# treangenlab/Seqwin

Measured on AMD Instinct MI355X. Metric: Gbp/s minimizer-indexed, higher is better.
Workload: dtype u64

## Files before the change

### seqwin_amd/csrc/device.hpp

```cpp
#pragma once

#include <hip/hip_runtime.h>

#include <functional>
#include <memory>
#include <string>

#include "common.hpp"

namespace sw {

#define SW_HIP(expr)                                                                                   \
    do {                                                                                               \
        hipError_t _e = (expr);                                                                        \
        if (_e != hipSuccess)                                                                          \
            ::sw::raise(SW_ERR_DEVICE, "HIP error %d (%s) at %s:%d: %s", (int)_e, hipGetErrorString(_e), \
                        __FILE__, __LINE__, #expr);                                                    \
    } while (0)

__host__ __device__ inline uint64_t mix64(uint64_t x)
{
    x ^= x >> 30; x *= 0xbf58476d1ce4e5b9ULL;
    x ^= x >> 27; x *= 0x94d049bb133111ebULL;
    x ^= x >> 31;
// ... 181 lines not shown
};
std::vector<int> devices_from_env();
void build_multi_device(const char *const *paths, size_t n_paths, uint64_t k, uint64_t w, uint64_t n_cpu, std::vector<int> devs,
                        MultiGraph &out, uint64_t chunk_bp = 0);

Plan &get_plan(sw_batch &b, uint64_t k, uint64_t w, bool *cached = nullptr);

struct SketchOut {
    DevArray<uint64_t> stage_hash;
    DevArray<uint64_t> stage_kmer;
    DevArray<uint32_t> tile_count;
    DevArray<uint64_t> tile_offset;
    uint64_t n_occ = 0;
    uint64_t launches = 0;
    uint64_t n_ovf_tiles = 0;
};
void run_sketch(const sw_batch &b, const Plan &plan, hipStream_t stream, SketchOut &out, float *sketch_ms);

void radix_sort_keys64(uint64_t *&keys, uint64_t *&alt, uint64_t n, unsigned begin_bit, unsigned end_bit, hipStream_t stream,
                       uint32_t *d_fail, bool perm_hi32 = false, unsigned long long *d_hist_given = nullptr, unsigned layout_bits = 0);
void radix_layout(unsigned bits, unsigned *digit_bits, unsigned *n_passes);
bool radix_unsort_perm(uint64_t *&keys, uint64_t *&alt, uint64_t n, unsigned low_bits, unsigned nbit, hipStream_t stream, uint32_t *d_fail);
constexpr uint32_t UNSORT_CURSOR_STRIDE = 32;
struct UnsortPerm {
    DevArray<unsigned long long> cur_a, cur_b;
    DevArray<uint32_t> tickets;
    unsigned low_bits = 0, hi_bits = 0;
    uint32_t n_groups = 0, n_tiles = 0, grid = 0;
};
bool radix_unsort_perm_begin(UnsortPerm &u, uint64_t n, unsigned low_bits, unsigned nbit, hipStream_t stream);
void radix_unsort_perm_first(UnsortPerm &u, const uint64_t *keys, uint64_t *alt, uint64_t n, hipStream_t stream, uint32_t *d_fail);
void radix_unsort_perm_second(UnsortPerm &u, const uint64_t *keys, uint64_t *alt, uint64_t n, hipStream_t stream, uint32_t *d_fail);

int radix_edge_buckets(uint64_t *&keys, uint64_t *&alt, uint64_t m, unsigned key_bits, uint64_t sentinel,
                       const unsigned long long *d_hist_top, uint32_t cap, uint32_t slots, uint64_t *ukeys, uint32_t *ucnt,
                       uint32_t *n_runs, hipStream_t stream, uint32_t *d_fail, bool debug);

void sort_keys64(uint64_t *&keys, uint64_t *&keys_alt, size_t n, unsigned begin_bit, unsigned end_bit, hipStream_t stream,
                 uint32_t *d_fail, bool perm_hi32 = false, unsigned long long *d_hist_given = nullptr, unsigned layout_bits = 0);
bool sort_keys64_is_own(size_t n);
void check_sort_failed(uint32_t fail_word);

struct alignas(16) OccPay {
    uint32_t low, pos, rec, idx;
};
int radix_rank_mode();
bool radix_pairs_available();
uint64_t radix_trim_state();
void radix_demote_rank();
constexpr uint32_t STAGE_WIN = 32;
constexpr uint32_t STAGE_ROW = STAGE_WIN + 9;
constexpr uint32_t STAGE_PAD = 1;
struct StageSource {
    const uint64_t *stage_hash, *stage_kmer;
    const uint32_t *tile_count;
    const uint64_t *tile_offset;
    const uint64_t *dst_off;
    uint32_t n_tiles;
    uint64_t mult;
    uint32_t *rec_out;
    const unsigned long long *chunk_dir;
    const uint64_t *rows;
};
void radix_sort_pairs32(uint32_t *&keys, uint32_t *&keys_alt, OccPay *&vals, OccPay *&vals_alt, uint64_t n, unsigned end_bit,
                        hipStream_t stream, uint32_t *d_fail, const StageSource *src = nullptr,
                        const std::function<void()> &after_first = std::function<void()>(), uint32_t *low_out = nullptr);
bool sort_pairs32(uint32_t *&keys, uint32_t *&keys_alt, OccPay *&vals, OccPay *&vals_alt, uint64_t n, unsigned end_bit,
                  hipStream_t stream, uint32_t *d_fail, uint32_t *low_out = nullptr);
struct PartState;
// ... 80 lines not shown
```

### seqwin_amd/csrc/index.hip

```cpp
#include <cstdlib>
#include <cstring>
#include <map>
#include <memory>

#include <rocprim/rocprim.hpp>

#include "device.hpp"

namespace sw {

namespace {

constexpr int TPB = 256;
inline unsigned blocks_for(uint64_t n, int per = TPB) { return (unsigned)((n + per - 1) / per); }
inline bool ranks_by_table()
{
    const char *e = SW_TEST_GETENV("SEQWIN_AMD_RANKS");
    return e && !strcmp(e, "table");
}

template <class K, class V>
void sort_pairs(K *&keys, K *&keys_alt, V *&vals, V *&vals_alt, size_t n, unsigned begin_bit, unsigned end_bit,
                hipStream_t stream)
{
// ... 1160 lines not shown
                                  unsigned hi_bits, uint64_t lo_base, const RankHash H, sw_edge *__restrict__ edges)
{
    const uint64_t e = (uint64_t)blockIdx.x * blockDim.x + threadIdx.x;
    if (e >= n_edges) return;
    const uint64_t key = ukeys[e];
    const uint64_t u = (hi_bits >= 64 ? 0ull : (key >> hi_bits)) + lo_base;
    const uint64_t v = hi_bits >= 64 ? key : (key & ((1ull << hi_bits) - 1ull));
    edges[e].first = H(u);
    edges[e].second = H(v);
    edges[e].weight = RUNS ? usum[e + 1] - usum[e] : usum[e];
}

struct RepeatFlag {
    const uint64_t *keys;
    const uint32_t *vals;
    __host__ __device__ uint32_t operator()(uint64_t s) const
    {
        return (s && keys[s] == keys[s - 1] && vals[s] == vals[s - 1]) ? 1u : 0u;
    }
};

__global__ void k_subtract_repeats(const uint64_t *__restrict__ rkeys, const uint32_t *__restrict__ rdups, uint32_t n_runs,
                                   const uint64_t *__restrict__ ukeys, uint64_t n_edges, sw_edge *__restrict__ edges)
{
    const uint32_t i = blockIdx.x * blockDim.x + threadIdx.x;
    if (i >= n_runs || rdups[i] == 0) return;
    const uint64_t key = rkeys[i];
    uint64_t lo = 0, hi = n_edges;
    while (lo < hi) {
        const uint64_t mid = (lo + hi) >> 1;
        if (ukeys[mid] < key) lo = mid + 1; else hi = mid;
    }
    if (lo < n_edges && ukeys[lo] == key) edges[lo].weight -= rdups[i];
}

struct AsmChangeAny {
    const uint64_t *keys;
    const uint32_t *vals;
    __host__ __device__ uint32_t operator()(uint64_t s) const
    {
        return (s == 0 || keys[s] != keys[s - 1] || vals[s] != vals[s - 1]) ? 1u : 0u;
    }
};

__global__ void k_check_ascending(const uint64_t *__restrict__ keys, uint64_t m, uint32_t *__restrict__ order_bad)
{
    const uint64_t i = (uint64_t)blockIdx.x * blockDim.x + threadIdx.x;
    if (i && i < m && keys[i] < keys[i - 1]) atomicAdd(order_bad, 1u);
}

__global__ void k_drop_sentinel_run(const uint64_t *__restrict__ ukeys, uint64_t sentinel, uint32_t *__restrict__ count)
{
    const uint32_t n = *count;
    if (n && ukeys[n - 1] == sentinel) *count = n - 1;
}

constexpr int RLE_THREADS = 1024, RLE_ITEMS = 8;
constexpr uint32_t RLE_TILE = RLE_THREADS * RLE_ITEMS;
__global__ __launch_bounds__(RLE_THREADS) void k_rle_keys(const uint64_t *__restrict__ keys, uint64_t m, uint64_t *__restrict__ ukeys,
                                                           uint32_t *__restrict__ ustart, unsigned long long *__restrict__ tile_state,
                                                           uint32_t *__restrict__ ticket, uint32_t *__restrict__ n_runs_out,
                                                           uint32_t *__restrict__ order_bad)
{
    __shared__ uint32_t s_tile, s_excl, s_wave[RLE_THREADS / 64];
    __shared__ uint64_t s_last[RLE_THREADS / 64];
    const uint32_t lane = threadIdx.x & 63u, wave = threadIdx.x >> 6;
// ... 1705 lines not shown
    SW_HIP(hipGetLastError());
    SW_HIP(hipStreamSynchronize(stream));
}
}

namespace {
constexpr uint64_t EDGE_BUCKET_MIN_KEYS = 1ull << 26;
constexpr uint32_t EDGE_BUCKET_CAP = 1u << 20, EDGE_BUCKET_SLOTS = 4096;
struct WideKeys {
    unsigned lo_bits, hi_bits;
    uint64_t lo_base;
    RankHash hash;
};
void edges_from_pairs(uint64_t *keys, uint64_t *keys_alt, uint64_t m, uint64_t sentinel, unsigned nb, unsigned ab,
                      uint64_t *ck, uint32_t *ca, const unsigned long long *d_n_cand, uint64_t host_n_cand,
                      const uint64_t *rank_hash, hipStream_t stream, sw_index &ix, hipEvent_t rank_hash_ready = nullptr,
                      unsigned long long *d_hist = nullptr, const WideKeys *wide = nullptr)
{
    ix.n_edges = 0;
    if (m == 0) return;
    const unsigned key_bits = wide ? wide->lo_bits + wide->hi_bits : 2 * nb;
    DevArray<uint32_t> sort_fail(1);
    SW_HIP(hipMemsetAsync(sort_fail.p, 0, 4, stream));
    unsigned low_bits = 0, skip = 0, digit_bits = 0, n_passes = 0;
    if (sort_keys64_is_own(m)) {
        radix_layout(key_bits, &digit_bits, &n_passes);
        const unsigned hb = wide ? wide->hi_bits : nb;
        skip = hb >= digit_bits + 8 ? 1 : 0;
        if (skip && hb >= 2 * digit_bits + 8 && ix.n_nodes && m <= 4 * ix.n_nodes) skip = 2;
        if (const char *e = SW_TEST_GETENV("SEQWIN_AMD_EDGE_SKIP_PASSES")) skip = (unsigned)atoi(e);
        skip = std::min(skip, n_passes - 1);
        low_bits = skip * digit_bits;
    }
    DevArray<uint64_t> ukeys(m);
    DevArray<uint32_t> ucnt(m + 1), ucount(2);
    unsigned long long n_cand = host_n_cand;
    const char *rle_env = SW_AB_GETENV("SEQWIN_AMD_RLE");
    const bool own_rle = !(rle_env && !strcmp(rle_env, "rocprim"));
    bool by_buckets = !wide && nb < 32 && own_rle && sort_keys64_is_own(m) && m >= EDGE_BUCKET_MIN_KEYS && ix.n_nodes && m > 4 * ix.n_nodes;
    uint32_t bucket_cap = EDGE_BUCKET_CAP, bucket_slots = EDGE_BUCKET_SLOTS;
    if (const char *e = SW_TEST_GETENV("SEQWIN_AMD_EDGE_SORT")) by_buckets = !wide && nb < 32 && own_rle && !strcmp(e, "bucket");
    if (const char *e = SW_TEST_GETENV("SEQWIN_AMD_EDGE_BUCKET_CAP")) bucket_cap = (uint32_t)strtoul(e, nullptr, 10);
    if (const char *e = SW_TEST_GETENV("SEQWIN_AMD_EDGE_BUCKET_SLOTS")) bucket_slots = (uint32_t)strtoul(e, nullptr, 10);
    if (by_buckets) {
        unsigned db = 0, np = 0;
        radix_layout(key_bits, &db, &np);
        uint32_t n_runs = 0;
        by_buckets = radix_edge_buckets(keys, keys_alt, m, key_bits, sentinel, d_hist ? d_hist + ((size_t)(np - 1) << db) : nullptr, bucket_cap,
                                        bucket_slots, ukeys.p, ucnt.p, &n_runs, stream, sort_fail.p,
                                        getenv("SEQWIN_AMD_DEBUG_EDGE_REPAIR") != nullptr) == 0;
        if (by_buckets) {
            uint32_t failed = 0;
            SW_HIP(hipMemcpyAsync(&failed, sort_fail.p, 4, hipMemcpyDeviceToHost, stream));
            if (d_n_cand) SW_HIP(hipMemcpyAsync(&n_cand, d_n_cand, 8, hipMemcpyDeviceToHost, stream));
            SW_HIP(hipStreamSynchronize(stream));
            check_sort_failed(failed);
            ix.n_edges = n_runs;
        }
    }
    if (!by_buckets)
        sort_keys64(keys, keys_alt, m, low_bits, key_bits, stream, sort_fail.p, false,
                    d_hist ? d_hist + ((size_t)skip << digit_bits) : nullptr, key_bits);
    RepairState rep;
    if (low_bits && !by_buckets) enqueue_repair(EdgeKeyView{keys, low_bits}, EdgeKeyView{keys, low_bits}, ~0ull, m, nullptr, 0, rep, stream);
    bool demoted = false;
    for (int attempt = 0; !by_buckets; ++attempt) {
        SW_HIP(hipMemsetAsync(ucount.p + 1, 0, 4, stream));
        if (own_rle) {
            const unsigned blocks = (unsigned)((m + RLE_TILE - 1) / RLE_TILE);
            DevArray<unsigned long long> tile_state(blocks);
            DevArray<uint32_t> ticket(1);
            SW_HIP(hipMemsetAsync(tile_state.p, 0, (size_t)blocks * 8, stream));
            SW_HIP(hipMemsetAsync(ticket.p, 0, 4, stream));
            hipLaunchKernelGGL(k_rle_keys, dim3(blocks), dim3(RLE_THREADS), 0, stream, (const uint64_t *)keys, m, ukeys.p, ucnt.p, tile_state.p,
                               ticket.p, ucount.p, ucount.p + 1);
            SW_HIP(hipGetLastError());
        } else {
#ifdef SW_AB
            hipLaunchKernelGGL(k_check_ascending, dim3(blocks_for(m)), dim3(TPB), 0, stream, (const uint64_t *)keys, m, ucount.p + 1);
            size_t tmp_bytes = 0;
            SW_HIP(rocprim::run_length_encode(nullptr, tmp_bytes, keys, m, ukeys.p, ucnt.p, ucount.p, stream));
            DevArray<unsigned char> tmp(tmp_bytes);
            SW_HIP(rocprim::run_length_encode(tmp.p, tmp_bytes, keys, m, ukeys.p, ucnt.p, ucount.p, stream));
            SW_HIP(hipStreamSynchronize(stream));
#endif
        }
        hipLaunchKernelGGL(k_drop_sentinel_run, dim3(1), dim3(1), 0, stream, ukeys.p, sentinel, ucount.p);
        SW_HIP(hipGetLastError());
        uint32_t n_edges = 0, failed = 0, left = 0, descents = 0;
        SW_HIP(hipMemcpyAsync(&n_edges, ucount.p, 4, hipMemcpyDeviceToHost, stream));
        SW_HIP(hipMemcpyAsync(&descents, ucount.p + 1, 4, hipMemcpyDeviceToHost, stream));
        SW_HIP(hipMemcpyAsync(&failed, sort_fail.p, 4, hipMemcpyDeviceToHost, stream));
        if (low_bits && attempt == 0) SW_HIP(hipMemcpyAsync(&left, rep.status.p, 4, hipMemcpyDeviceToHost, stream));
        if (d_n_cand) SW_HIP(hipMemcpyAsync(&n_cand, d_n_cand, 8, hipMemcpyDeviceToHost, stream));
        SW_HIP(hipStreamSynchronize(stream));
        check_sort_failed(failed);
        if (low_bits && attempt == 0 && getenv("SEQWIN_AMD_DEBUG_EDGE_REPAIR")) {
            unsigned long long nd[2] = {0, 0};
            uint32_t st[2] = {0, 0};
            SW_HIP(hipMemcpy(nd, rep.n_desc.p, 16, hipMemcpyDeviceToHost));
            SW_HIP(hipMemcpy(st, rep.status.p, 8, hipMemcpyDeviceToHost));
            fprintf(stderr, "[edge repair] %llu keys, %u low bits: %llu descents, %u long runs, leftovers %u\n", (unsigned long long)m, low_bits,
                    nd[0], st[1], st[0]);
        }
        if (left) {
            sort_keys64(keys, keys_alt, m, 0, key_bits, stream, sort_fail.p);
            continue;
        }
        if (descents) {
            if (demoted)
                raise(SW_ERR_RUNTIME, "internal error: the edge keys are still out of order after the ballot-ranked re-sort (%u places)", descents);
            order_guard_tripped(1, descents);
            radix_demote_rank();
            demoted = true;
            sort_keys64(keys, keys_alt, m, 0, key_bits, stream, sort_fail.p);
            continue;
        }
        ix.n_edges = n_edges;
        break;
    }
    if (ix.n_edges == 0) return;
    ix.edges.alloc(ix.n_edges);
    if (rank_hash_ready) SW_HIP(hipStreamWaitEvent(stream, rank_hash_ready, 0));
    if (wide && own_rle)
        hipLaunchKernelGGL(k_edges_runs_wide<true>, dim3(blocks_for(ix.n_edges)), dim3(TPB), 0, stream, ukeys.p, ucnt.p, (uint64_t)ix.n_edges,
                           wide->hi_bits, wide->lo_base, wide->hash, ix.edges.p);
    else if (wide)
        hipLaunchKernelGGL(k_edges_runs_wide<false>, dim3(blocks_for(ix.n_edges)), dim3(TPB), 0, stream, ukeys.p, ucnt.p, (uint64_t)ix.n_edges,
                           wide->hi_bits, wide->lo_base, wide->hash, ix.edges.p);
    else if (own_rle)
        hipLaunchKernelGGL(k_edges_runs<true>, dim3(blocks_for(ix.n_edges)), dim3(TPB), 0, stream, ukeys.p, ucnt.p, 0u, ~0ull,
                           (uint64_t)ix.n_edges, nb, ix.nodes.p, rank_hash, ix.edges.p);
    else
        hipLaunchKernelGGL(k_edges_runs<false>, dim3(blocks_for(ix.n_edges)), dim3(TPB), 0, stream, ukeys.p, ucnt.p, 0u, ~0ull,
                           (uint64_t)ix.n_edges, nb, ix.nodes.p, rank_hash, ix.edges.p);
    SW_HIP(hipGetLastError());
    if (n_cand) {
        const uint64_t c = n_cand;
        DevArray<uint64_t> ck1(c);
        DevArray<uint32_t> ca1(c);
        uint32_t *a = ca, *a_alt = ca1.p;
        uint64_t *k = ck, *k_alt = ck1.p;
        sort_pairs(a, a_alt, k, k_alt, c, 0, ab, stream);
        sort_pairs(k, k_alt, a, a_alt, c, 0, key_bits, stream);
        DevArray<uint64_t> rkeys(c);
        DevArray<uint32_t> rdups(c), rcount(1);
        auto flags = rocprim::make_transform_iterator(rocprim::make_counting_iterator<uint64_t>(0), RepeatFlag{k, a});
        size_t tmp_bytes = 0;
        SW_HIP(rocprim::reduce_by_key(nullptr, tmp_bytes, k, flags, c, rkeys.p, rdups.p, rcount.p, rocprim::plus<uint32_t>(),
                                      rocprim::equal_to<uint64_t>(), stream));
        DevArray<unsigned char> tmp(tmp_bytes);
        SW_HIP(rocprim::reduce_by_key(tmp.p, tmp_bytes, k, flags, c, rkeys.p, rdups.p, rcount.p, rocprim::plus<uint32_t>(),
                                      rocprim::equal_to<uint64_t>(), stream));
        uint32_t n_runs = 0;
        SW_HIP(hipMemcpyAsync(&n_runs, rcount.p, 4, hipMemcpyDeviceToHost, stream));
        SW_HIP(hipStreamSynchronize(stream));
        if (n_runs) {
            hipLaunchKernelGGL(k_subtract_repeats, dim3(blocks_for(n_runs)), dim3(TPB), 0, stream, rkeys.p, rdups.p, n_runs, ukeys.p,
                               (uint64_t)ix.n_edges, ix.edges.p);
            SW_HIP(hipGetLastError());
        }
    }
    SW_HIP(hipStreamSynchronize(stream));
}

void edges_from_adjacency(uint64_t *keys, uint64_t *keys_alt, uint32_t *vals, uint32_t *vals_alt, uint64_t m,
                          uint64_t sentinel, unsigned nb, const uint64_t *rank_hash, hipStream_t stream, sw_index &ix)
{
    ix.n_edges = 0;
    if (m == 0) return;
    sort_pairs(keys, keys_alt, vals, vals_alt, m, 0, 2 * nb, stream);
    DevArray<uint64_t> ukeys(m);
    DevArray<uint32_t> usum(m);
    DevArray<uint32_t> ucount(1);
    {
        auto flags = rocprim::make_transform_iterator(rocprim::make_counting_iterator<uint64_t>(0), AsmChangeAny{keys, vals});
        size_t tmp_bytes = 0;
        SW_HIP(rocprim::reduce_by_key(nullptr, tmp_bytes, keys, flags, m, ukeys.p, usum.p, ucount.p, rocprim::plus<uint32_t>(),
                                      rocprim::equal_to<uint64_t>(), stream));
        DevArray<unsigned char> tmp(tmp_bytes);
        SW_HIP(rocprim::reduce_by_key(tmp.p, tmp_bytes, keys, flags, m, ukeys.p, usum.p, ucount.p, rocprim::plus<uint32_t>(),
                                      rocprim::equal_to<uint64_t>(), stream));
        hipLaunchKernelGGL(k_drop_sentinel_run, dim3(1), dim3(1), 0, stream, ukeys.p, sentinel, ucount.p);
        SW_HIP(hipGetLastError());
        uint32_t n_edges = 0;
        SW_HIP(hipMemcpyAsync(&n_edges, ucount.p, 4, hipMemcpyDeviceToHost, stream));
        SW_HIP(hipStreamSynchronize(stream));
        ix.n_edges = n_edges;
    }
    if (ix.n_edges == 0) return;
    ix.edges.alloc(ix.n_edges);
    hipLaunchKernelGGL(k_edges_runs<false>, dim3(blocks_for(ix.n_edges)), dim3(TPB), 0, stream, ukeys.p, usum.p, 0u, ~0ull,
                       (uint64_t)ix.n_edges, nb, ix.nodes.p, rank_hash, ix.edges.p);
    SW_HIP(hipGetLastError());
    SW_HIP(hipStreamSynchronize(stream));
}
// ... 1028 lines not shown
```

### seqwin_amd/csrc/radix.hip

```cpp
#include <algorithm>
#include <cstdlib>
#include <cstring>
#include <vector>
#include <map>
#include <mutex>

#include "device.hpp"

namespace sw {
namespace {

constexpr int RS_ITEMS = 16;
#ifdef SW_RS_STAMPS
__device__ unsigned long long *g_rs_stamps = nullptr;
#define RS_STAMP(i)                                                                                        \
    do {                                                                                                   \
        if (g_rs_stamps && (tile & 63u) == 0 && threadIdx.x == 0) g_rs_stamps[(size_t)(tile >> 6) * 16 + (i)] = clock64(); \
    } while (0)
#else
#define RS_STAMP(i) do { } while (0)
#endif
#ifndef RS_LOOK
#define RS_LOOK 4
#endif
// ... 1427 lines not shown
    }
}

#ifdef SW_RS_STAMPS
__device__ unsigned long long *g_eb_stamps = nullptr;
constexpr uint32_t EB_ST_EVERY = 16, EB_ST_WORDS = 16;
#define EB_STAMP(i) do { if (st) st[i] = clock64(); } while (0)
#define EB_STAMP_ADD(i, since) do { if (st) { const unsigned long long t_ = clock64(); st[i] += t_ - (since); (since) = t_; } } while (0)
#else
#define EB_STAMP(i) do { } while (0)
#define EB_STAMP_ADD(i, since) do { } while (0)
#endif

template <bool PACKED>
__global__ __launch_bounds__(EB_THREADS) void k_eb_finish(const uint64_t *__restrict__ in, const uint4 *__restrict__ live, uint32_t slots,
                                                          unsigned shift1, unsigned shift2, uint32_t mask2, unsigned bin_shift,
                                                          uint32_t bin_mask, unsigned cb, uint64_t sentinel,
                                                          uint64_t *__restrict__ tk, uint32_t *__restrict__ tc,
                                                          uint32_t *__restrict__ n_distinct, uint32_t *__restrict__ flags)
{
    extern __shared__ __align__(16) unsigned char eb_lds[];
    unsigned long long *hk = reinterpret_cast<unsigned long long *>(eb_lds);
    uint32_t *hc = reinterpret_cast<uint32_t *>(hk + slots);
    uint16_t *idx = PACKED ? reinterpret_cast<uint16_t *>(hk + slots) : reinterpret_cast<uint16_t *>(hc + slots);
    __shared__ uint32_t bd[EB_RADIX + 1], bk[EB_RADIX], bcur[EB_RADIX], wsd[EB_THREADS / 64], wsk[EB_THREADS / 64];
    __shared__ uint32_t s_over;
    const uint32_t tid = threadIdx.x, lane = tid & 63u, wave = tid >> 6;
#ifdef SW_RS_STAMPS
    unsigned long long *st = g_eb_stamps && tid == 0 && blockIdx.x % EB_ST_EVERY == 0 ? g_eb_stamps + (size_t)(blockIdx.x / EB_ST_EVERY) * EB_ST_WORDS : nullptr;
    unsigned long long st_t = 0;
#endif
    EB_STAMP(0);
    const uint4 me = live[blockIdx.x];
    const uint32_t mask = slots - 1u;
    for (uint32_t s = tid; s < slots; s += EB_THREADS) {
        hk[s] = EB_EMPTY;
        if (!PACKED) hc[s] = 0;
    }
    bd[tid] = 0;
    bk[tid] = 0;
    if (tid == 0) s_over = 0;
    const uint32_t b = me.x, first = me.y, cnt = me.z;
    const uint64_t low_mask = (1ull << shift2) - 1ull, count_mask = (1ull << cb) - 1ull;
    const uint64_t high = ((uint64_t)(b / EB_RADIX) << shift1) | ((uint64_t)(b % EB_RADIX) << shift2);
    uint64_t nxt[4];
#pragma unroll
    for (int i = 0; i < 4; ++i) {
        const uint32_t j = i * EB_THREADS + tid;
        nxt[i] = j < cnt ? in[(uint64_t)first + j] : sentinel;
    }
    EB_STAMP(1);
    __syncthreads();
    EB_STAMP(2);
#ifdef SW_RS_STAMPS
    if (st) st_t = clock64();
#endif
    uint32_t bad = 0;
    for (uint32_t j0 = 0; j0 < cnt; j0 += 4 * EB_THREADS) {
        if (*(volatile uint32_t *)&s_over) break;
        uint64_t key[4];
#pragma unroll
        for (int i = 0; i < 4; ++i) key[i] = nxt[i];
        if (j0 + 4 * EB_THREADS < cnt) {
#pragma unroll
            for (int i = 0; i < 4; ++i) {
                const uint32_t j = j0 + 4 * EB_THREADS + i * EB_THREADS + tid;
                nxt[i] = j < cnt ? in[(uint64_t)first + j] : sentinel;
            }
        }
        uint32_t cp[4], h[4];
        unsigned long long w[4];
#pragma unroll
        for (int i = 0; i < 4; ++i) {
            const uint64_t k = key[i];
            bool alive = k != sentinel;
            if (alive && ((uint32_t)(k >> shift1) * EB_RADIX + ((uint32_t)(k >> shift2) & mask2)) != b) {
                bad = 1;
                alive = false;
            }
            uint32_t copies = 1;
            const uint64_t any = __ballot(alive);
            if (any) {
                const int src = __ffsll((long long)any) - 1;
                const uint64_t k0 = (uint64_t)__shfl((unsigned long long)k, src, 64);
                const uint64_t same = __ballot(alive && k == k0);
                if (alive && k == k0) {
                    copies = (uint32_t)__popcll(same);
                    alive = (int)lane == src;
                }
            }
            cp[i] = alive ? copies : 0u;
            h[i] = (uint32_t)((k * 0x9E3779B97F4A7C15ull) >> 40) & mask;
            w[i] = PACKED ? ((k & low_mask) << cb) | copies : (unsigned long long)k;
        }
        EB_STAMP_ADD(3, st_t);
        for (uint32_t probes = 0; cp[0] | cp[1] | cp[2] | cp[3]; ++probes) {
            if (probes == slots) {
                s_over = 1;
                break;
            }
            unsigned long long old[4];
#pragma unroll
            for (int i = 0; i < 4; ++i)
                if (cp[i]) old[i] = atomicCAS(&hk[h[i]], EB_EMPTY, w[i]);
#pragma unroll
            for (int i = 0; i < 4; ++i) {
                if (!cp[i]) continue;
                if (PACKED) {
                    if (old[i] == EB_EMPTY) cp[i] = 0;
                    else if ((old[i] >> cb) == (w[i] >> cb)) {
                        atomicAdd(&hk[h[i]], (unsigned long long)cp[i]);
                        cp[i] = 0;
                    } else h[i] = (h[i] + 1u) & mask;
                } else {
                    if (old[i] == EB_EMPTY || old[i] == w[i]) {
                        atomicAdd(&hc[h[i]], cp[i]);
                        cp[i] = 0;
                    } else h[i] = (h[i] + 1u) & mask;
                }
            }
        }
        EB_STAMP_ADD(4, st_t);
    }
    if (bad) atomicOr(flags, EB_F_RANGE);
    __syncthreads();
    EB_STAMP(5);
    if (s_over) {
        if (tid == 0) atomicOr(flags, EB_F_OVERFLOW);
        return;
    }
    const unsigned wbin_shift = PACKED ? bin_shift + cb : bin_shift;
    for (uint32_t s = tid; s < slots; s += EB_THREADS) {
        const uint64_t k = hk[s];
        if (k == EB_EMPTY) continue;
        const uint32_t bin = (uint32_t)(k >> wbin_shift) & bin_mask;
        atomicAdd(&bd[bin], 1u);
        atomicAdd(&bk[bin], PACKED ? (uint32_t)(k & count_mask) : hc[s]);
    }
    __syncthreads();
    EB_STAMP(6);
    {
        const uint32_t d = bd[tid], c = bk[tid];
        uint32_t id = d, ic = c;
        for (uint32_t o = 1; o < 64; o <<= 1) {
            const uint32_t ud = __shfl_up(id, o, 64), uc = __shfl_up(ic, o, 64);
            if (lane >= o) {
                id += ud;
                ic += uc;
            }
        }
        if (lane == 63) {
            wsd[wave] = id;
            wsk[wave] = ic;
        }
        __syncthreads();
        uint32_t pd = id - d, pc = ic - c;
        for (uint32_t w2 = 0; w2 < wave; ++w2) {
            pd += wsd[w2];
            pc += wsk[w2];
        }
        bd[tid] = pd;
        bcur[tid] = pd;
        bk[tid] = pc;
// ... 40 lines not shown
#ifdef SW_RS_STAMPS
    if (st) {
        st[9] = clock64();
        st[10] = cnt;
        st[11] = n_dist;
    }
#endif
}

__global__ __launch_bounds__(256) void k_eb_compact(const uint64_t *__restrict__ tk, const uint32_t *__restrict__ tc,
                                                    const uint4 *__restrict__ live, uint32_t n_live, const uint32_t *__restrict__ start,
                                                    const uint32_t *__restrict__ dstart,
                                                    const unsigned long long *__restrict__ n_sentinels, uint64_t *__restrict__ ukeys,
                                                    uint32_t *__restrict__ ucnt, uint32_t *__restrict__ flags)
{
    if (blockIdx.x == 0 && threadIdx.x == 0) ucnt[dstart[EB_TABLE]] = start[EB_TABLE] - (uint32_t)*n_sentinels;
    if (blockIdx.x >= n_live) return;
    const uint4 me = live[blockIdx.x];
    const uint32_t b = me.x, d0 = dstart[b], n = dstart[b + 1] - d0;
    if (n == 0) return;
    const uint64_t first = me.y;
    const uint32_t end = me.y + me.z;
    uint32_t bad = 0;
    for (uint32_t j = threadIdx.x; j < n; j += 256) {
        const uint64_t k = tk[first + j];
        const uint32_t c = tc[first + j];
        if (j + 1 < n && (tk[first + j + 1] <= k || tc[first + j + 1] <= c)) bad = 1;
        if (c < first || c >= end) bad = 1;
        ukeys[d0 + j] = k;
        ucnt[d0 + j] = c;
    }
    if (bad) atomicOr(flags, EB_F_ORDER);
}
}

int radix_edge_buckets(uint64_t *&keys, uint64_t *&alt, uint64_t m, unsigned key_bits, uint64_t sentinel,
                       const unsigned long long *d_hist_top, uint32_t cap, uint32_t slots, uint64_t *ukeys, uint32_t *ucnt,
                       uint32_t *n_runs, hipStream_t stream, uint32_t *d_fail, bool debug)
{
    constexpr int THREADS = 1024, BITS = 9;
    constexpr uint32_t TILE = THREADS * RS_ITEMS;
    unsigned digit_bits = 0, n_passes = 0;
    radix_layout(key_bits, &digit_bits, &n_passes);
    if (n_passes < 2 || m >= (1ull << 32) - 1 || slots < 64 || slots > 8192 || (slots & (slots - 1))) return 1;
    const unsigned shift1 = (n_passes - 1) * digit_bits, bits1 = key_bits - shift1;
    const unsigned bits2 = std::min<unsigned>(BITS, shift1), shift2 = shift1 - bits2;
    const unsigned bin_bits = std::min<unsigned>(BITS, shift2), bin_shift = shift2 - bin_bits;
    const uint64_t n_tiles = (m + TILE - 1) / TILE, max_tiles2 = n_tiles + EB_RADIX;
    int dev = 0, per_cu = 0;
    SW_HIP(hipGetDevice(&dev));
    hipDeviceProp_t prop;
    SW_HIP(hipGetDeviceProperties(&prop, dev));
    SW_HIP(hipOccupancyMaxActiveBlocksPerMultiprocessor(&per_cu, k_rs_pass_p<THREADS, BITS, 0>, THREADS, 0));
    const unsigned cus = (unsigned)std::max(1, prop.multiProcessorCount);
    const unsigned grid = (unsigned)std::min<uint64_t>(n_tiles, (uint64_t)std::max(1, per_cu) * cus);

    DevArray<unsigned long long> h1(EB_RADIX), cur1((size_t)EB_RADIX * RS_CURSOR_STRIDE), cur2(EB_TABLE), segtab(max_tiles2);
    DevArray<uint32_t> table(EB_TABLE), start(EB_TABLE + 1), tickets(2), flags(1);
    DevArray<uint4> live(EB_TABLE);
    DevArray<EbInfo> info(1);
    SW_HIP(hipMemsetAsync(h1.p, 0, h1.bytes(), stream));
    SW_HIP(hipMemsetAsync(table.p, 0, table.bytes(), stream));
    SW_HIP(hipMemsetAsync(tickets.p, 0, 8, stream));
    SW_HIP(hipMemsetAsync(flags.p, 0, 4, stream));
    SW_HIP(hipMemsetAsync(info.p, 0, sizeof(EbInfo), stream));
    if (d_hist_top)
        SW_HIP(hipMemcpyAsync(h1.p, d_hist_top, (size_t)8 << digit_bits, hipMemcpyDeviceToDevice, stream));
    else
        hipLaunchKernelGGL(k_rs_hist<BITS>, dim3((unsigned)((m + 32767) / 32768)), dim3(256), 0, stream, (const uint64_t *)keys, m, shift1,
                           key_bits, 1u, h1.p);
    hipLaunchKernelGGL(k_eb_level1, dim3(1), dim3(EB_RADIX), 0, stream, (const unsigned long long *)h1.p, TILE, cur1.p, segtab.p, info.p);
// ... 59 lines not shown
        hipLaunchKernelGGL(finish, dim3(hi.n_live), dim3(EB_THREADS), lds, stream, (const uint64_t *)keys, (const uint4 *)live.p, slots, shift1,
                           shift2, (1u << bits2) - 1u, bin_shift, (1u << bin_bits) - 1u, cb, sentinel, tk, tc.p, n_distinct.p, flags.p);
#ifdef SW_RS_STAMPS
    if (stamps.p) {
        std::vector<unsigned long long> hs(n_st);
        SW_HIP(hipStreamSynchronize(stream));
        SW_HIP(hipMemcpy(hs.data(), stamps.p, stamps.bytes(), hipMemcpyDeviceToHost));
        unsigned long long *none = nullptr;
        SW_HIP(hipMemcpyToSymbol(HIP_SYMBOL(g_eb_stamps), &none, sizeof none));
        double acc[10] = {0}, keys_sum = 0, dist_sum = 0;
        size_t cnt = 0;
        for (size_t t = 0; t + EB_ST_WORDS <= n_st; t += EB_ST_WORDS) {
            if (!hs[t] || !hs[t + 9] || hs[t + 10] <= 2 * 4 * EB_THREADS || hs[t + 10] > 3 * 4 * EB_THREADS) continue;
            acc[1] += (double)(hs[t + 1] - hs[t]);
            acc[2] += (double)(hs[t + 2] - hs[t + 1]);
            acc[3] += (double)hs[t + 3];
            acc[4] += (double)hs[t + 4];
            acc[5] += (double)(hs[t + 5] - hs[t + 2]) - (double)hs[t + 3] - (double)hs[t + 4];
            for (int i = 6; i <= 9; ++i) acc[i] += (double)(hs[t + i] - hs[t + i - 1]);
            keys_sum += (double)hs[t + 10];
            dist_sum += (double)hs[t + 11];
            ++cnt;
        }
        static const char *nm[] = {"", "entry+list", "init+barrier", "merge(+key wait)", "probes", "loop barrier", "bin count", "scan", "scatter", "rank+store"};
        fprintf(stderr, "[eb stamps] %s slots, %zu workgroups of 3 steps sampled (mean %.0f keys, %.0f distinct); mean clocks:", packed ? "packed" : "plain",
                cnt, cnt ? keys_sum / cnt : 0.0, cnt ? dist_sum / cnt : 0.0);
        double sum = 0;
        for (int i = 1; i <= 9; ++i) { fprintf(stderr, " %s=%.0f", nm[i], cnt ? acc[i] / cnt : 0.0); sum += cnt ? acc[i] / cnt : 0.0; }
        fprintf(stderr, " | workgroup %.0f\n", sum);
    }
#endif
    hipLaunchKernelGGL(k_eb_scan, dim3(1), dim3(1024), 0, stream, (const uint32_t *)n_distinct.p, (const unsigned long long *)nullptr, 0u,
                       dstart.p, (unsigned long long *)nullptr, (uint32_t *)nullptr, &info.p->n_runs, (uint4 *)nullptr, (uint32_t *)nullptr);
    hipLaunchKernelGGL(k_eb_compact, dim3(std::max(1u, hi.n_live)), dim3(256), 0, stream, (const uint64_t *)tk, (const uint32_t *)tc.p,
                       (const uint4 *)live.p, hi.n_live, (const uint32_t *)start.p, (const uint32_t *)dstart.p,
                       (const unsigned long long *)&info.p->n_sentinels, ukeys, ucnt, flags.p);
    SW_HIP(hipGetLastError());
    uint32_t hf = 0;
    SW_HIP(hipMemcpyAsync(&hi, info.p, sizeof hi, hipMemcpyDeviceToHost, stream));
    SW_HIP(hipMemcpyAsync(&hf, flags.p, 4, hipMemcpyDeviceToHost, stream));
    SW_HIP(hipStreamSynchronize(stream));
    if (hf & (EB_F_RANGE | EB_F_ORDER))
        raise(SW_ERR_RUNTIME, "internal error: the edge buckets are out of order (%s)", hf & EB_F_RANGE ? "a key outside its bucket" : "run starts descend");
    if (hf & EB_F_OVERFLOW) {
        if (debug) fprintf(stderr, "[edge buckets] a sub-bucket holds more than %u distinct keys: radix passes instead\n", slots);
        return 1;
    }
    *n_runs = hi.n_runs;
    return 0;
}

static int pick_shape(unsigned bits)
{
    const char *e = SW_TEST_GETENV("SEQWIN_AMD_RADIX_BITS");
    const bool nine = e ? atoi(e) == 9 : (bits + 8) / 9 < (bits + 7) / 8;
    const char *shape = SW_AB_GETENV("SEQWIN_AMD_RADIX_SHAPE");
    if (shape && !strcmp(shape, "1024x8")) return 2;
    if (shape && !strcmp(shape, "512x9")) return 3;
    if (shape && !strcmp(shape, "256x8")) return 4;
    return nine ? 1 : 0;
}

void radix_layout(unsigned bits, unsigned *digit_bits, unsigned *n_passes)
{
    const int sh = pick_shape(bits);
    *digit_bits = (sh == 1 || sh == 3) ? 9u : 8u;
    *n_passes = (bits + *digit_bits - 1) / *digit_bits;
}

void radix_sort_keys64(uint64_t *&keys, uint64_t *&alt, uint64_t n, unsigned begin_bit, unsigned end_bit, hipStream_t stream,
                       uint32_t *d_fail, bool perm_hi32, unsigned long long *d_hist_given, unsigned layout_bits)
{
    if (n == 0 || end_bit <= begin_bit) return;
    if (end_bit - begin_bit > 64) raise(SW_ERR_RUNTIME, "radix_sort_keys64: more than 64 key bits");
    switch (pick_shape(layout_bits ? layout_bits : end_bit - begin_bit)) {
#ifdef SW_AB
    case 2: sort_passes<1024, 8>(keys, alt, n, begin_bit, end_bit, stream, d_fail, perm_hi32, d_hist_given); break;
    case 3: sort_passes<512, 9>(keys, alt, n, begin_bit, end_bit, stream, d_fail, perm_hi32, d_hist_given); break;
    case 4: sort_passes<256, 8>(keys, alt, n, begin_bit, end_bit, stream, d_fail, perm_hi32, d_hist_given); break;
#endif
    case 1: sort_passes<1024, 9>(keys, alt, n, begin_bit, end_bit, stream, d_fail, perm_hi32, d_hist_given); break;
    default: sort_passes<512, 8>(keys, alt, n, begin_bit, end_bit, stream, d_fail, perm_hi32, d_hist_given); break;
// ... 5 lines not shown
```

Measured before the change: 493.4.

## Emit edges directly from edge sub-buckets, skipping the compact pass

When the bucketed edge sort runs and a rank hash is available, the compact kernel that writes unique keys and counts is skipped. A new kernel builds edges straight from the sub-bucket tables, hashing both endpoints and staging rows through LDS for vectorized stores. The ukeys/ucnt arrays are no longer allocated on this path, host readbacks are merged into a single synchronization, and the repeat-subtraction kernel now binary-searches on the hashed edge pairs. The sub-bucket kernel also polls a global overflow flag so other workgroups can stop early, at the cost of an extra atomic load per step.

After: 495.7 (median of 6 runs). Within noise of the previous version (+0.5%).

```diff
diff --git a/seqwin_amd/csrc/device.hpp b/seqwin_amd/csrc/device.hpp
--- a/seqwin_amd/csrc/device.hpp
+++ b/seqwin_amd/csrc/device.hpp
@@ -237,9 +237,19 @@
 void radix_unsort_perm_first(UnsortPerm &u, const uint64_t *keys, uint64_t *alt, uint64_t n, hipStream_t stream, uint32_t *d_fail);
 void radix_unsort_perm_second(UnsortPerm &u, const uint64_t *keys, uint64_t *alt, uint64_t n, hipStream_t stream, uint32_t *d_fail);
 
+struct EdgeBuckets {
+    const uint64_t *tk = nullptr;
+    DevArray<uint32_t> tc, start, dstart, flags;
+    DevArray<uint4> live;
+    uint32_t n_live = 0;
+    unsigned long long n_sentinels = 0;
+    std::function<void()> before_sync;
+};
 int radix_edge_buckets(uint64_t *&keys, uint64_t *&alt, uint64_t m, unsigned key_bits, uint64_t sentinel,
                        const unsigned long long *d_hist_top, uint32_t cap, uint32_t slots, uint64_t *ukeys, uint32_t *ucnt,
-                       uint32_t *n_runs, hipStream_t stream, uint32_t *d_fail, bool debug);
+                       uint32_t *n_runs, hipStream_t stream, uint32_t *d_fail, bool debug, EdgeBuckets *stop = nullptr);
+void radix_edge_buckets_emit(const EdgeBuckets &eb, unsigned nb, const uint64_t *rank_hash, sw_edge *edges, hipStream_t stream);
+void radix_edge_buckets_order(const EdgeBuckets &eb, hipStream_t stream);
 
 void sort_keys64(uint64_t *&keys, uint64_t *&keys_alt, size_t n, unsigned begin_bit, unsigned end_bit, hipStream_t stream,
                  uint32_t *d_fail, bool perm_hi32 = false, unsigned long long *d_hist_given = nullptr, unsigned layout_bits = 0);
diff --git a/seqwin_amd/csrc/index.hip b/seqwin_amd/csrc/index.hip
--- a/seqwin_amd/csrc/index.hip
+++ b/seqwin_amd/csrc/index.hip
@@ -1216,6 +1216,20 @@
         if (ukeys[mid] < key) lo = mid + 1; else hi = mid;
     }
     if (lo < n_edges && ukeys[lo] == key) edges[lo].weight -= rdups[i];
+}
+
+__global__ void k_subtract_repeats_hash(const uint64_t *__restrict__ rkeys, const uint32_t *__restrict__ rdups, uint32_t n_runs, unsigned nb,
+                                        const uint64_t *__restrict__ rank_hash, uint64_t n_edges, sw_edge *__restrict__ edges)
+{
+    const uint32_t i = blockIdx.x * blockDim.x + threadIdx.x;
+    if (i >= n_runs || rdups[i] == 0) return;
+    const uint64_t key = rkeys[i], hu = rank_hash[key >> nb], hv = rank_hash[key & ((1ull << nb) - 1ull)];
+    uint64_t lo = 0, hi = n_edges;
+    while (lo < hi) {
+        const uint64_t mid = (lo + hi) >> 1, f = edges[mid].first;
+        if (f < hu || (f == hu && edges[mid].second < hv)) lo = mid + 1; else hi = mid;
+    }
+    if (lo < n_edges && edges[lo].first == hu && edges[lo].second == hv) edges[lo].weight -= rdups[i];
 }
 
 struct AsmChangeAny {
@@ -2987,8 +3001,8 @@
         skip = std::min(skip, n_passes - 1);
         low_bits = skip * digit_bits;
     }
-    DevArray<uint64_t> ukeys(m);
-    DevArray<uint32_t> ucnt(m + 1), ucount(2);
+    DevArray<uint64_t> ukeys;
+    DevArray<uint32_t> ucnt, ucount(2);
     unsigned long long n_cand = host_n_cand;
     const char *rle_env = SW_AB_GETENV("SEQWIN_AMD_RLE");
     const bool own_rle = !(rle_env && !strcmp(rle_env, "rocprim"));
@@ -2997,25 +3011,43 @@
     if (const char *e = SW_TEST_GETENV("SEQWIN_AMD_EDGE_SORT")) by_buckets = !wide && nb < 32 && own_rle && !strcmp(e, "bucket");
     if (const char *e = SW_TEST_GETENV("SEQWIN_AMD_EDGE_BUCKET_CAP")) bucket_cap = (uint32_t)strtoul(e, nullptr, 10);
     if (const char *e = SW_TEST_GETENV("SEQWIN_AMD_EDGE_BUCKET_SLOTS")) bucket_slots = (uint32_t)strtoul(e, nullptr, 10);
+    EdgeBuckets eb;
+    bool fused = by_buckets && rank_hash;
+    if (const char *e = SW_TEST_GETENV("SEQWIN_AMD_EDGE_EMIT")) fused = fused && strcmp(e, "compact") != 0;
     if (by_buckets) {
         unsigned db = 0, np = 0;
         radix_layout(key_bits, &db, &np);
-        uint32_t n_runs = 0;
+        uint32_t n_runs = 0, failed = 0;
+        const bool debug = getenv("SEQWIN_AMD_DEBUG_EDGE_REPAIR") != nullptr;
+        if (fused) {
+            eb.before_sync = [&] {
+                SW_HIP(hipMemcpyAsync(&failed, sort_fail.p, 4, hipMemcpyDeviceToHost, stream));
+                if (d_n_cand) SW_HIP(hipMemcpyAsync(&n_cand, d_n_cand, 8, hipMemcpyDeviceToHost, stream));
+            };
+        } else {
+            ukeys.alloc(m);
+            ucnt.alloc(m + 1);
+        }
         by_buckets = radix_edge_buckets(keys, keys_alt, m, key_bits, sentinel, d_hist ? d_hist + ((size_t)(np - 1) << db) : nullptr, bucket_cap,
-                                        bucket_slots, ukeys.p, ucnt.p, &n_runs, stream, sort_fail.p,
-                                        getenv("SEQWIN_AMD_DEBUG_EDGE_REPAIR") != nullptr) == 0;
+                                        bucket_slots, ukeys.p, ucnt.p, &n_runs, stream, sort_fail.p, debug, fused ? &eb : nullptr) == 0;
         if (by_buckets) {
-            uint32_t failed = 0;
-            SW_HIP(hipMemcpyAsync(&failed, sort_fail.p, 4, hipMemcpyDeviceToHost, stream));
-            if (d_n_cand) SW_HIP(hipMemcpyAsync(&n_cand, d_n_cand, 8, hipMemcpyDeviceToHost, stream));
-            SW_HIP(hipStreamSynchronize(stream));
+            if (!fused) {
+                SW_HIP(hipMemcpyAsync(&failed, sort_fail.p, 4, hipMemcpyDeviceToHost, stream));
+                if (d_n_cand) SW_HIP(hipMemcpyAsync(&n_cand, d_n_cand, 8, hipMemcpyDeviceToHost, stream));
+                SW_HIP(hipStreamSynchronize(stream));
+            }
             check_sort_failed(failed);
             ix.n_edges = n_runs;
-        }
-    }
-    if (!by_buckets)
+            if (debug) fprintf(stderr, "[edge buckets] edges written %s\n", fused ? "from the sub-buckets (fused)" : "from the run arrays (compact)");
+        }
+    }
+    fused = fused && by_buckets;
+    if (!by_buckets) {
+        if (!ukeys.p) ukeys.alloc(m);
+        if (!ucnt.p) ucnt.alloc(m + 1);
         sort_keys64(keys, keys_alt, m, low_bits, key_bits, stream, sort_fail.p, false,
                     d_hist ? d_hist + ((size_t)skip << digit_bits) : nullptr, key_bits);
+    }
     RepairState rep;
     if (low_bits && !by_buckets) enqueue_repair(EdgeKeyView{keys, low_bits}, EdgeKeyView{keys, low_bits}, ~0ull, m, nullptr, 0, rep, stream);
     bool demoted = false;
@@ -3077,7 +3109,9 @@
     if (ix.n_edges == 0) return;
     ix.edges.alloc(ix.n_edges);
     if (rank_hash_ready) SW_HIP(hipStreamWaitEvent(stream, rank_hash_ready, 0));
-    if (wide && own_rle)
+    if (fused)
+        radix_edge_buckets_emit(eb, nb, rank_hash, ix.edges.p, stream);
+    else if (wide && own_rle)
         hipLaunchKernelGGL(k_edges_runs_wide<true>, dim3(blocks_for(ix.n_edges)), dim3(TPB), 0, stream, ukeys.p, ucnt.p, (uint64_t)ix.n_edges,
                            wide->hi_bits, wide->lo_base, wide->hash, ix.edges.p);
     else if (wide)
@@ -3111,12 +3145,19 @@
         SW_HIP(hipMemcpyAsync(&n_runs, rcount.p, 4, hipMemcpyDeviceToHost, stream));
         SW_HIP(hipStreamSynchronize(stream));
         if (n_runs) {
-            hipLaunchKernelGGL(k_subtract_repeats, dim3(blocks_for(n_runs)), dim3(TPB), 0, stream, rkeys.p, rdups.p, n_runs, ukeys.p,
-                               (uint64_t)ix.n_edges, ix.edges.p);
+            if (fused)
+                hipLaunchKernelGGL(k_subtract_repeats_hash, dim3(blocks_for(n_runs)), dim3(TPB), 0, stream, rkeys.p, rdups.p, n_runs, nb,
+                                   rank_hash, (uint64_t)ix.n_edges, ix.edges.p);
+            else
+                hipLaunchKernelGGL(k_subtract_repeats, dim3(blocks_for(n_runs)), dim3(TPB), 0, stream, rkeys.p, rdups.p, n_runs, ukeys.p,
+                                   (uint64_t)ix.n_edges, ix.edges.p);
             SW_HIP(hipGetLastError());
         }
     }
-    SW_HIP(hipStreamSynchronize(stream));
+    if (fused)
+        radix_edge_buckets_order(eb, stream);
+    else
+        SW_HIP(hipStreamSynchronize(stream));
 }
 
 void edges_from_adjacency(uint64_t *keys, uint64_t *keys_alt, uint32_t *vals, uint32_t *vals_alt, uint64_t m,
diff --git a/seqwin_amd/csrc/radix.hip b/seqwin_amd/csrc/radix.hip
--- a/seqwin_amd/csrc/radix.hip
+++ b/seqwin_amd/csrc/radix.hip
@@ -1483,6 +1483,7 @@
 #endif
     EB_STAMP(0);
     const uint4 me = live[blockIdx.x];
+    uint32_t seen = __hip_atomic_load(flags, __ATOMIC_RELAXED, __HIP_MEMORY_SCOPE_AGENT);
     const uint32_t mask = slots - 1u;
     for (uint32_t s = tid; s < slots; s += EB_THREADS) {
         hk[s] = EB_EMPTY;
@@ -1508,7 +1509,8 @@
 #endif
     uint32_t bad = 0;
     for (uint32_t j0 = 0; j0 < cnt; j0 += 4 * EB_THREADS) {
-        if (*(volatile uint32_t *)&s_over) break;
+        if (seen & EB_F_OVERFLOW) s_over = 2;
+        if ((seen & EB_F_OVERFLOW) || *(volatile uint32_t *)&s_over) break;
         uint64_t key[4];
 #pragma unroll
         for (int i = 0; i < 4; ++i) key[i] = nxt[i];
@@ -1518,6 +1520,7 @@
                 const uint32_t j = j0 + 4 * EB_THREADS + i * EB_THREADS + tid;
                 nxt[i] = j < cnt ? in[(uint64_t)first + j] : sentinel;
             }
+            seen = __hip_atomic_load(flags, __ATOMIC_RELAXED, __HIP_MEMORY_SCOPE_AGENT);
         }
         uint32_t cp[4], h[4];
         unsigned long long w[4];
@@ -1548,6 +1551,7 @@
         for (uint32_t probes = 0; cp[0] | cp[1] | cp[2] | cp[3]; ++probes) {
             if (probes == slots) {
                 s_over = 1;
+                atomicOr(flags, EB_F_OVERFLOW);
                 break;
             }
             unsigned long long old[4];
@@ -1576,10 +1580,7 @@
     if (bad) atomicOr(flags, EB_F_RANGE);
     __syncthreads();
     EB_STAMP(5);
-    if (s_over) {
-        if (tid == 0) atomicOr(flags, EB_F_OVERFLOW);
-        return;
-    }
+    if (s_over) return;
     const unsigned wbin_shift = PACKED ? bin_shift + cb : bin_shift;
     for (uint32_t s = tid; s < slots; s += EB_THREADS) {
         const uint64_t k = hk[s];
@@ -1686,11 +1687,77 @@
     }
     if (bad) atomicOr(flags, EB_F_ORDER);
 }
+
+constexpr uint32_t EE_THREADS = 256, EE_ITEMS = 4, EE_STAGE = EE_THREADS * EE_ITEMS;
+static_assert(sizeof(sw_edge) == 24, "k_eb_edges stages an edge as three 8-byte words");
+__global__ __launch_bounds__(EE_THREADS) void k_eb_edges(const uint64_t *__restrict__ tk, const uint32_t *__restrict__ tc,
+                                                          const uint4 *__restrict__ live, const uint32_t *__restrict__ start,
+                                                          const uint32_t *__restrict__ dstart, uint32_t n_sentinels, unsigned nb,
+                                                          const uint64_t *__restrict__ rank_hash, sw_edge *__restrict__ edges,
+                                                          uint32_t *__restrict__ flags)
+{
+    __shared__ __align__(16) unsigned long long stage[3 * EE_STAGE];
+    const uint4 me = live[blockIdx.x];
+    const uint32_t b = me.x, d0 = dstart[b], n = dstart[b + 1] - d0;
+    if (n == 0) return;
+    const uint32_t tid = threadIdx.x, lane = tid & 63u;
+    const uint64_t first = me.y, mask = (1ull << nb) - 1ull;
+    const uint32_t end = me.y + me.z, total = start[EB_TABLE], last_end = end == total ? end - n_sentinels : end;
+    unsigned long long *out = reinterpret_cast<unsigned long long *>(edges);
+    uint32_t bad = 0;
+    for (uint32_t c0 = 0; c0 < n; c0 += EE_STAGE) {
+        uint64_t k[EE_ITEMS], nk[EE_ITEMS];
+        uint32_t c[EE_ITEMS], nc[EE_ITEMS];
+#pragma unroll
+        for (uint32_t i = 0; i < EE_ITEMS; ++i) {
+            const uint32_t j = c0 + i * EE_THREADS + tid;
+            const bool own = lane == 63 && j + 1 < n;
+            k[i] = j < n ? tk[first + j] : 0ull;
+            c[i] = j < n ? tc[first + j] : 0u;
+            nk[i] = own ? tk[first + j + 1] : 0ull;
+            nc[i] = own ? tc[first + j + 1] : 0u;
+        }
+        uint64_t hu[EE_ITEMS], hv[EE_ITEMS];
+#pragma unroll
+        for (uint32_t i = 0; i < EE_ITEMS; ++i) {
+            const uint32_t j = c0 + i * EE_THREADS + tid;
+            hu[i] = j < n ? rank_hash[k[i] >> nb] : 0ull;
+            hv[i] = j < n ? rank_hash[k[i] & mask] : 0ull;
+        }
+#pragma unroll
+        for (uint32_t i = 0; i < EE_ITEMS; ++i) {
+            const uint32_t l = i * EE_THREADS + tid, j = c0 + l;
+            uint64_t kn = (uint64_t)__shfl_down((unsigned long long)k[i], 1, 64);
+            uint32_t cn = __shfl_down(c[i], 1, 64);
+            if (lane == 63) {
+                kn = nk[i];
+                cn = nc[i];
+            }
+            if (j >= n) continue;
+            const bool more = j + 1 < n;
+            if (more && (kn <= k[i] || cn <= c[i])) bad = 1;
+            if (c[i] < first || c[i] >= end) bad = 1;
+            stage[3 * l] = hu[i];
+            stage[3 * l + 1] = hv[i];
+            stage[3 * l + 2] = (uint32_t)((more ? cn : last_end) - c[i]);
+        }
+        __syncthreads();
+        const uint32_t words = 3u * min(EE_STAGE, n - c0);
+        const uint64_t w0 = 3ull * ((uint64_t)d0 + c0);
+        const uint32_t head = (uint32_t)(w0 & 1ull), pairs = (words - head) / 2u;
+        if (head && tid == 0) out[w0] = stage[0];
+        for (uint32_t p = tid; p < pairs; p += EE_THREADS)
+            *reinterpret_cast<ulonglong2 *>(out + w0 + head + 2u * p) = make_ulonglong2(stage[head + 2u * p], stage[head + 2u * p + 1u]);
+        if (((words - head) & 1u) && tid == EE_THREADS - 1) out[w0 + words - 1u] = stage[words - 1u];
+        __syncthreads();
+    }
+    if (bad) atomicOr(flags, EB_F_ORDER);
+}
 }
 
 int radix_edge_buckets(uint64_t *&keys, uint64_t *&alt, uint64_t m, unsigned key_bits, uint64_t sentinel,
                        const unsigned long long *d_hist_top, uint32_t cap, uint32_t slots, uint64_t *ukeys, uint32_t *ucnt,
-                       uint32_t *n_runs, hipStream_t stream, uint32_t *d_fail, bool debug)
+                       uint32_t *n_runs, hipStream_t stream, uint32_t *d_fail, bool debug, EdgeBuckets *stop)
 {
     constexpr int THREADS = 1024, BITS = 9;
     constexpr uint32_t TILE = THREADS * RS_ITEMS;
@@ -1816,13 +1883,17 @@
 #endif
     hipLaunchKernelGGL(k_eb_scan, dim3(1), dim3(1024), 0, stream, (const uint32_t *)n_distinct.p, (const unsigned long long *)nullptr, 0u,
                        dstart.p, (unsigned long long *)nullptr, (uint32_t *)nullptr, &info.p->n_runs, (uint4 *)nullptr, (uint32_t *)nullptr);
-    hipLaunchKernelGGL(k_eb_compact, dim3(std::max(1u, hi.n_live)), dim3(256), 0, stream, (const uint64_t *)tk, (const uint32_t *)tc.p,
-                       (const uint4 *)live.p, hi.n_live, (const uint32_t *)start.p, (const uint32_t *)dstart.p,
-                       (const unsigned long long *)&info.p->n_sentinels, ukeys, ucnt, flags.p);
+    if (!stop)
+        hipLaunchKernelGGL(k_eb_compact, dim3(std::max(1u, hi.n_live)), dim3(256), 0, stream, (const uint64_t *)tk, (const uint32_t *)tc.p,
+                           (const uint4 *)live.p, hi.n_live, (const uint32_t *)start.p, (const uint32_t *)dstart.p,
+                           (const unsigned long long *)&info.p->n_sentinels, ukeys, ucnt, flags.p);
     SW_HIP(hipGetLastError());
     uint32_t hf = 0;
+    const uint32_t n_live = hi.n_live;
+    const unsigned long long n_sentinels = hi.n_sentinels;
     SW_HIP(hipMemcpyAsync(&hi, info.p, sizeof hi, hipMemcpyDeviceToHost, stream));
     SW_HIP(hipMemcpyAsync(&hf, flags.p, 4, hipMemcpyDeviceToHost, stream));
+    if (stop && stop->before_sync) stop->before_sync();
     SW_HIP(hipStreamSynchronize(stream));
     if (hf & (EB_F_RANGE | EB_F_ORDER))
         raise(SW_ERR_RUNTIME, "internal error: the edge buckets are out of order (%s)", hf & EB_F_RANGE ? "a key outside its bucket" : "run starts descend");
@@ -1831,7 +1902,33 @@
         return 1;
     }
     *n_runs = hi.n_runs;
+    if (stop) {
+        stop->tk = tk;
+        stop->tc = std::move(tc);
+        stop->start = std::move(start);
+        stop->dstart = std::move(dstart);
+        stop->flags = std::move(flags);
+        stop->live = std::move(live);
+        stop->n_live = n_live;
+        stop->n_sentinels = n_sentinels;
+    }
     return 0;
+}
+
+void radix_edge_buckets_emit(const EdgeBuckets &eb, unsigned nb, const uint64_t *rank_hash, sw_edge *edges, hipStream_t stream)
+{
+    if (!eb.n_live) return;
+    hipLaunchKernelGGL(k_eb_edges, dim3(eb.n_live), dim3(EE_THREADS), 0, stream, eb.tk, (const uint32_t *)eb.tc.p, (const uint4 *)eb.live.p,
+                       (const uint32_t *)eb.start.p, (const uint32_t *)eb.dstart.p, (uint32_t)eb.n_sentinels, nb, rank_hash, edges, eb.flags.p);
+    SW_HIP(hipGetLastError());
+}
+
+void radix_edge_buckets_order(const EdgeBuckets &eb, hipStream_t stream)
+{
+    uint32_t hf = 0;
+    SW_HIP(hipMemcpyAsync(&hf, eb.flags.p, 4, hipMemcpyDeviceToHost, stream));
+    SW_HIP(hipStreamSynchronize(stream));
+    if (hf & EB_F_ORDER) raise(SW_ERR_RUNTIME, "internal error: the edge buckets are out of order (%s)", "run starts descend");
 }
 
 static int pick_shape(unsigned bits)
```
